# chaoting-sun/GCT-Plus

Hardware: AMD Instinct MI355X
Metric: SMILES/sec training step (vaetf, seq_len=80, d_model=512) (higher is better)
Workload: dtype f32

## Files before the change

gct_plus_amd/csrc/gemm.hip:

```cpp
#include <limits.h>
#include <stdlib.h>

#include <type_traits>

#include "common.h"

typedef float f32x16 __attribute__((ext_vector_type(16)));

namespace {

constexpr int BM = 128, BN = 128, BK = 32;
constexpr int TILE_FLOATS = BM * BK;

struct Seg3 {
  const float* p0;
  int64_t d1, d2;
};

struct GemmArgs {
  int64_t M, N, K;
  Seg3 a;
  int64_t lda;
  int64_t a_nper;
  Seg3 b;
// ... 930 lines not shown
#pragma unroll
    for (int rr = 0; rr < 4; ++rr) v[rr] = *reinterpret_cast<const float4*>(stg + (rg * 4 + rr) * 32 + c4 * 4);
    if (g.epi == EPI_SLAB) {
      float* sl = g.c0 + (int64_t)z * g.slab_stride;
#pragma unroll
      for (int rr = 0; rr < 4; ++rr)
        if (row0 + rr < g.M) *reinterpret_cast<float4*>(sl + (row0 + rr) * g.N + col0) = v[rr];
      return;
    }
    const bool q1 = col0 >= g.c_nper, q2 = col0 >= 2 * g.c_nper;
    const int64_t cloc = col0 - (q2 ? 2 * g.c_nper : (q1 ? g.c_nper : 0));
    float* cbase = g.c0 + (q2 ? g.c_d2 : (q1 ? g.c_d1 : 0));
    float4 bias = make_float4(0.f, 0.f, 0.f, 0.f);
    if (g.bias0) bias = *reinterpret_cast<const float4*>(g.bias0 + (q2 ? g.bias_d2 : (q1 ? g.bias_d1 : 0)) + cloc);
    ep.apply(v, row0, col0, cbase, cloc, bias);
  }
}


template <int TN, bool RAGGED = false>
__global__ __launch_bounds__(256) void gemm_f32_panel_kernel(const GemmArgs g) {
  constexpr int TM = 32, KC = 256, SD = KC + 4, NBL = TN / 4;
  extern __shared__ __attribute__((aligned(16))) float plds[];
  float* As = plds;
  float* Bs = plds + TM * SD;
  const int tid = threadIdx.x, lane = tid & 63, wave = tid >> 6, g4 = lane >> 4, c16 = lane & 15;
  const unsigned tiles_m = (unsigned)((g.M + TM - 1) / TM);
  const unsigned lid = gct_xcd_remap(blockIdx.x, gridDim.x);
  const int64_t m0 = (int64_t)(lid % tiles_m) * TM, n0 = (int64_t)(lid / tiles_m) * TN;
  const bool s1 = n0 >= g.b_nper, s2 = n0 >= 2 * g.b_nper;
  const float* bbase = g.b.p0 + (s2 ? g.b.d2 : (s1 ? g.b.d1 : 0)) + (n0 - (s2 ? 2 * g.b_nper : (s1 ? g.b_nper : 0))) * g.ldb;
  const float* abase = g.a.p0;
  uint32_t offa[8], offb[NBL];
#pragma unroll
  for (int i = 0; i < 8; ++i) {
    const int idx = tid + 256 * i, row = idx >> 6, c4 = idx & 63;
    int64_t r = m0 + row;
    if (r > g.M - 1) r = g.M - 1;
    offa[i] = (uint32_t)(r * g.lda + c4 * 4);
  }
#pragma unroll
  for (int i = 0; i < NBL; ++i) {
    const int idx = tid + 256 * i, c4 = idx & 63;
    int64_t row = idx >> 6;
    if (RAGGED && n0 + row > g.N - 1) row = g.N - 1 - n0;
    offb[i] = (uint32_t)(row * g.ldb + c4 * 4);
  }
  f32x4_t ra[8], rb[NBL];
  auto gload = [&](int64_t k0) {
#pragma unroll
    for (int i = 0; i < 8; ++i) ra[i] = *reinterpret_cast<const f32x4_t*>(abase + k0 + offa[i]);
#pragma unroll
    for (int i = 0; i < NBL; ++i) rb[i] = *reinterpret_cast<const f32x4_t*>(bbase + k0 + offb[i]);
  };
  auto lstore = [&]() {
#pragma unroll
    for (int i = 0; i < 8; ++i) {
      const int idx = tid + 256 * i;
      *reinterpret_cast<f32x4_t*>(As + (idx >> 6) * SD + (idx & 63) * 4) = ra[i];
    }
#pragma unroll
    for (int i = 0; i < NBL; ++i) {
      const int idx = tid + 256 * i;
      *reinterpret_cast<f32x4_t*>(Bs + (idx >> 6) * SD + (idx & 63) * 4) = rb[i];
    }
  };
  constexpr int NS = TN / 32;
  const int wm = (wave >> 1) * 16, wn = (wave & 1) * (TN / 2);
  f32x4_t acc[NS];
#pragma unroll
  for (int j = 0; j < NS; ++j) acc[j] = (f32x4_t){0.f, 0.f, 0.f, 0.f};
  const int64_t nch = g.K / KC;
  gload(0);
  lstore();
  __syncthreads();
  for (int64_t c = 0; c < nch; ++c) {
    if (c + 1 < nch) gload((c + 1) * KC);
    const float* ap = As + (wm + c16) * SD + g4 * 64;
#pragma unroll 4
    for (int j = 0; j < 16; ++j) {
      const float4 a4 = *reinterpret_cast<const float4*>(ap + 4 * j);
#pragma unroll
      for (int u = 0; u < NS; ++u) {
        const float4 b4 = *reinterpret_cast<const float4*>(Bs + (wn + 16 * u + c16) * SD + g4 * 64 + 4 * j);
        acc[u] = __builtin_amdgcn_mfma_f32_16x16x4f32(a4.x, b4.x, acc[u], 0, 0, 0);
        acc[u] = __builtin_amdgcn_mfma_f32_16x16x4f32(a4.y, b4.y, acc[u], 0, 0, 0);
        acc[u] = __builtin_amdgcn_mfma_f32_16x16x4f32(a4.z, b4.z, acc[u], 0, 0, 0);
        acc[u] = __builtin_amdgcn_mfma_f32_16x16x4f32(a4.w, b4.w, acc[u], 0, 0, 0);
      }
    }
    __syncthreads();
    if (c + 1 < nch) {
      lstore();
      __syncthreads();
    }
  }
  float* stg = plds + wave * (16 * 20);
  const FastEpi ep{g};
#pragma unroll
  for (int u = 0; u < NS; ++u) {
#pragma unroll
    for (int i = 0; i < 4; ++i) stg[(4 * g4 + i) * 20 + c16] = acc[u][i];
    __builtin_amdgcn_s_waitcnt(0xC07F);
    __builtin_amdgcn_wave_barrier();
    if (lane < 16) {
      const int pr = lane >> 2, pc = lane & 3;
      const int64_t row0 = m0 + wm + 4 * pr, col0 = n0 + wn + 16 * u + 4 * pc;
      if (RAGGED) {
        for (int rr = 0; rr < 4; ++rr)
          for (int cc = 0; cc < 4; ++cc)
            if (row0 + rr < g.M && col0 + cc < g.N)
              g.c0[(row0 + rr) * g.ldc + col0 + cc] = stg[(4 * pr + rr) * 20 + 4 * pc + cc] + (g.bias0 ? g.bias0[col0 + cc] : 0.f);
      } else if (row0 < g.M && col0 < g.N) {
        float4 v[4];
#pragma unroll
        for (int rr = 0; rr < 4; ++rr) v[rr] = *reinterpret_cast<const float4*>(stg + (4 * pr + rr) * 20 + 4 * pc);
        const bool q1 = col0 >= g.c_nper, q2 = col0 >= 2 * g.c_nper;
        const int64_t cloc = col0 - (q2 ? 2 * g.c_nper : (q1 ? g.c_nper : 0));
        float* cbase = g.c0 + (q2 ? g.c_d2 : (q1 ? g.c_d1 : 0));
        float4 bias = make_float4(0.f, 0.f, 0.f, 0.f);
        if (g.bias0) bias = *reinterpret_cast<const float4*>(g.bias0 + (q2 ? g.bias_d2 : (q1 ? g.bias_d1 : 0)) + cloc);
        ep.apply(v, row0, col0, cbase, cloc, bias);
      }
    }
    __builtin_amdgcn_s_waitcnt(0xC07F);
    __builtin_amdgcn_wave_barrier();
  }
}

template <int TN, bool RAGGED = false>
int launch_panel(const GemmArgs& g, hipStream_t st) {
  constexpr size_t LDS = (size_t)(32 + TN) * 260 * sizeof(float);
  static bool attr_set = false;
  if (!attr_set) {
    hipError_t e = hipFuncSetAttribute((const void*)gemm_f32_panel_kernel<TN, RAGGED>, hipFuncAttributeMaxDynamicSharedMemorySize, (int)LDS);
    if (e != hipSuccess) {
      gct_set_error("gemm_f32_panel: cannot reserve %zu bytes of LDS: %s", LDS, hipGetErrorString(e));
      return GCT_ERR_HIP;
    }
    attr_set = true;
  }
  const int64_t tiles = ((g.M + 31) / 32) * (RAGGED ? 1 : g.N / TN);
  hipLaunchKernelGGL((gemm_f32_panel_kernel<TN, RAGGED>), dim3((unsigned)tiles), dim3(256), LDS, st, g);
  GCT_LAUNCH_CHECK("gemm_f32_panel");
  return GCT_OK;
}

__global__ __launch_bounds__(256) void splitk_epilogue_kernel(const GemmArgs g, const float* slabs,
                                                              int nslab, int64_t slab_stride) {
  const int64_t pc = g.N / 4, pr = (g.M + 3) / 4;
  const int64_t idx = (int64_t)blockIdx.x * blockDim.x + threadIdx.x;
  if (idx >= pc * pr) return;
  const int64_t row0 = (idx / pc) * 4, col0 = (idx % pc) * 4;
  float4 v[4];
#pragma unroll
  for (int rr = 0; rr < 4; ++rr) {
    v[rr] = make_float4(0.f, 0.f, 0.f, 0.f);
    if (row0 + rr < g.M) {
      const float* p = slabs + (row0 + rr) * g.N + col0;
      for (int s = 0; s < nslab; ++s) {
        const float4 t = *reinterpret_cast<const float4*>(p + (int64_t)s * slab_stride);
        v[rr].x += t.x; v[rr].y += t.y; v[rr].z += t.z; v[rr].w += t.w;
      }
    }
  }
  const bool q1 = col0 >= g.c_nper, q2 = col0 >= 2 * g.c_nper;
  const int64_t cloc = col0 - (q2 ? 2 * g.c_nper : (q1 ? g.c_nper : 0));
  float* cbase = g.c0 + (q2 ? g.c_d2 : (q1 ? g.c_d1 : 0));
  float4 bias = make_float4(0.f, 0.f, 0.f, 0.f);
  if (g.bias0) bias = *reinterpret_cast<const float4*>(g.bias0 + (q2 ? g.bias_d2 : (q1 ? g.bias_d1 : 0)) + cloc);
  const FastEpi ep{g};
  ep.apply(v, row0, col0, cbase, cloc, bias);
}

int g_gemm_mode = -1;
int64_t g_gemm_launches[2] = {0, 0};
inline int gemm_mode() {
  if (g_gemm_mode < 0) {
    const char* e = getenv("GCT_GEMM_MODE");
    g_gemm_mode = (e && (e[0] == 'f' || e[0] == '0')) ? GCT_GEMM_F32 : GCT_GEMM_BF16X6;
  }
  return g_gemm_mode;
}

template <bool A_KC, bool B_KC>
bool fast_ok(const GemmArgs& g, bool vec) {
  auto seg_ok = [](int64_t nper, int64_t extent, int64_t gran) { return nper >= extent || nper % gran == 0; };
  return vec && g.K % BK == 0 && g.ksplit % BK == 0 && g.M >= 4 && g.N >= 4 &&
         (A_KC ? seg_ok(g.a_nper, g.K, BK) : (seg_ok(g.a_nper, g.M, BM) && g.M % 4 == 0)) &&
         (B_KC ? seg_ok(g.b_nper, g.N, BN) : (seg_ok(g.b_nper, g.K, BK) && g.N % 4 == 0)) &&
         g.N % 4 == 0 && g.ldc % 4 == 0 && gct_aligned16(g.c0) && g.c_d1 % 4 == 0 && g.c_d2 % 4 == 0 &&
         (g.c_nper >= g.N || g.c_nper % 4 == 0) && g.slab_stride % 4 == 0 &&
         (!g.bias0 || (gct_aligned16(g.bias0) && g.bias_d1 % 4 == 0 && g.bias_d2 % 4 == 0)) &&
         (!g.resid || gct_aligned16(g.resid)) && (!g.pre || gct_aligned16(g.pre)) &&
         (!g.pre_in || gct_aligned16(g.pre_in)) && 130 * g.lda < (1ll << 31) && 130 * g.ldb < (1ll << 31);
}


inline int64_t slab_bytes(int64_t s, int64_t rows, int64_t cols) {
  return s > 1 ? s * rows * cols * (int64_t)sizeof(float) : 0;
}

inline bool skinny_m(int64_t M, int64_t N) { return ((M + BM - 1) / BM) * ((N + BN - 1) / BN) < 192; }

int skinny_splits(int64_t M, int64_t N, int64_t K) {
  const int64_t tiles = ((M + 63) / 64) * ((N + 63) / 64);
  if (tiles <= 0) return 1;
  int64_t ns = 768 / tiles;
  if (ns > K / BK / 4) ns = K / BK / 4;
  return ns < 1 ? 1 : (int)ns;
}

int x6_tail_plan(int64_t M, int64_t N, int64_t K, int64_t* m1_out) {
  constexpr int64_t CUS = 256;
  const int64_t tm = (M + XBM - 1) / XBM, tn = (N + XBN - 1) / XBN, tiles = tm * tn;
  const int64_t rem = tiles % CUS;
  if (tiles <= CUS || rem == 0 || rem % tn != 0 || K % XBK != 0) return 1;
  const int64_t nkt = K / XBK;
  int best = 1;
  double cost = 1.0;
  const double o = 3.3;
  for (int s2 = 2; s2 <= 8 && nkt / s2 >= 2; ++s2) {
    const double c = (double)((rem * s2 + CUS - 1) / CUS) * (o + (double)nkt / s2) / (o + nkt) + 0.05;
    if (c < cost - 1e-9) { cost = c; best = s2; }
  }
  if (best == 1 || cost > 0.75) return 1;
  *m1_out = (tiles - rem) / tn * XBM;
  return best;
}

int x6_splitk_all_plan(int64_t M, int64_t N, int64_t K) {
  constexpr int64_t CUS = 256;
  const int64_t tiles = ((M + XBM - 1) / XBM) * ((N + XBN - 1) / XBN), nkt = K / XBK;
  if (tiles > CUS / 2 || K % XBK != 0 || nkt < 32 || M < 1024 || (nkt < 64 && M < 2048)) return 1;
  int64_t sp = CUS / tiles;
  if (sp > nkt / 8) sp = nkt / 8;
  if (sp > 8) sp = 8;
  return sp < 2 ? 1 : (int)sp;
}


inline int64_t x6s_tiles(int64_t M, int64_t N) { return ((M + SBM - 1) / SBM) * ((N + SBN - 1) / SBN); }

inline bool x6s_shape(const GemmArgs& g) {
  const int64_t big = ((g.M + XBM - 1) / XBM) * ((g.N + XBN - 1) / XBN), small = x6s_tiles(g.M, g.N), nkt = g.K / XBK;
  return big <= 160 && small >= 96 && small <= (nkt <= 16 ? 512 : 256) && nkt <= 32;
}

constexpr int64_t X6_TAIL_SMALL_MAX = 512;

constexpr int64_t PANEL32_MAX_TILES = 4096, PANEL64_MAX_TILES = 768;


static_assert(BK == XBK, "the fp32 and bf16x6 kernels split K at the same granularity");
GemmArgs slab_args(const GemmArgs& g, int splits, float* ws) {
  const int64_t nkt = g.K / BK;
  GemmArgs p = g;
  p.ksplit = ((nkt + splits - 1) / splits) * BK;
  p.nsplit = (int)((g.K + p.ksplit - 1) / p.ksplit);
  p.epi = EPI_SLAB; p.c0 = ws; p.ldc = g.N; p.slab_stride = g.M * g.N;
  p.c_d1 = p.c_d2 = 0; p.c_nper = INT64_MAX / 4; p.bias0 = nullptr; p.resid = nullptr; p.pre = nullptr; p.pre_in = nullptr;
  return p;
}

int launch_fixup(const GemmArgs& g, const GemmArgs& slabs, hipStream_t st, const char* name) {
  const int64_t patches = ((g.M + 3) / 4) * (g.N / 4);
  hipLaunchKernelGGL(splitk_epilogue_kernel, dim3((unsigned)((patches + 255) / 256)), dim3(256), 0, st, g,
                     (const float*)slabs.c0, slabs.nsplit, slabs.slab_stride);
  GCT_LAUNCH_CHECK(name);
  return GCT_OK;
}

template <int MODE, int NP>
int launch_x6_tail_split(const GemmArgs& g, hipStream_t st, float* ws, int64_t ws_bytes) {
  if (MODE == X6_WGRAD || g.nsplit != 1 || !ws || !gct_aligned16(ws)) return launch_x6<MODE, NP>(g, st);
  int64_t m1 = 0;
  const int best = x6_tail_plan(g.M, g.N, g.K, &m1);
  const int64_t m2 = g.M - m1, nkt = g.K / XBK;
  hipStreamCaptureStatus cap = hipStreamCaptureStatusNone;
  if (best == 1 || slab_bytes(best, m2, g.N) > ws_bytes ||
      hipStreamIsCapturing(st, &cap) != hipSuccess || cap != hipStreamCaptureStatusNone)
    return launch_x6<MODE, NP>(g, st);
  GemmArgs head = g;
  head.M = m1;
  int rc = launch_x6<MODE, NP>(head, st);
  if (rc) return rc;
  GemmArgs e = g;
  e.M = m2; e.row_base = g.row_base + m1;
  e.a.p0 += m1 * g.lda;
  e.c0 += m1 * g.ldc;
  if (e.resid) e.resid += m1 * g.ldc;
  if (e.pre) e.pre += m1 * g.ldc;
  if (e.pre_in && !(g.pre_rows > 0 && g.quad_map)) e.pre_in += m1 * g.ldc;
  if (nkt <= 32 && x6s_tiles(m2, g.N) <= X6_TAIL_SMALL_MAX) {
    if (MODE == X6_FWD && x6s_ok(e, true)) return launch_x6s<X6_FWD, NP>(e, st);
    if (MODE == X6_DGRAD && x6s_dgrad_ok(e, true)) return launch_x6s<X6_DGRAD, NP>(e, st);
  }
  const GemmArgs p = slab_args(e, best, ws);
  rc = launch_x6<MODE, NP>(p, st);
  if (rc) return rc;
  return launch_fixup(e, p, st, "x6 tail fix-up");
}

struct GemmRoute {
  enum Kind {
    X6S,
    X6_SPLITK_ALL,
    PANEL_THIN,
    PANEL32,
    PANEL64,
    F32_SMALL,
    X6,
    F32_FAST,
    F32_VEC,
    F32,
  } kind;
  int splits;
// ... 312 lines not shown
```

gct_plus_amd/csrc/norm.hip:

```cpp
#include "common.h"

namespace {

constexpr int MAXC = 8;

template <int NC>
__global__ __launch_bounds__(256) void norm_fwd_kernel(const float* __restrict__ x,
                                                       const float* __restrict__ alpha,
                                                       const float* __restrict__ bias, float* y,
                                                       float* mean_out, float* rstd_out,
                                                       int64_t rows, int d, float eps) {
  const int lane = threadIdx.x & 63, wave = threadIdx.x >> 6;
  const int64_t nwaves = (int64_t)gridDim.x * 4;
  float4 a[NC], b[NC];
#pragma unroll
  for (int c = 0; c < NC; ++c) {
    const int col = c * 256 + lane * 4;
    if (col < d) {
      a[c] = *reinterpret_cast<const float4*>(alpha + col);
      b[c] = *reinterpret_cast<const float4*>(bias + col);
    }
  }
  for (int64_t row = (int64_t)blockIdx.x * 4 + wave; row < rows; row += nwaves) {
    const float* xr = x + row * d;
    float4 v[NC];
    float s = 0.f;
#pragma unroll
    for (int c = 0; c < NC; ++c) {
      const int col = c * 256 + lane * 4;
      v[c] = make_float4(0.f, 0.f, 0.f, 0.f);
      if (col < d) {
        v[c] = *reinterpret_cast<const float4*>(xr + col);
        s += (v[c].x + v[c].y) + (v[c].z + v[c].w);
      }
    }
    const float mean = gct_wave_sum(s) / (float)d;
    float ss = 0.f;
#pragma unroll
    for (int c = 0; c < NC; ++c) {
      const int col = c * 256 + lane * 4;
      if (col < d) {
        v[c].x -= mean; v[c].y -= mean; v[c].z -= mean; v[c].w -= mean;
        ss += (v[c].x * v[c].x + v[c].y * v[c].y) + (v[c].z * v[c].z + v[c].w * v[c].w);
      }
    }
    const float var = gct_wave_sum(ss) / (float)(d - 1);
    const float rstd = 1.0f / (sqrtf(var) + eps);
    if (lane == 0) {
      mean_out[row] = mean;
      rstd_out[row] = rstd;
    }
    float* yr = y + row * d;
#pragma unroll
    for (int c = 0; c < NC; ++c) {
      const int col = c * 256 + lane * 4;
      if (col < d) {
        float4 o;
        o.x = a[c].x * (v[c].x * rstd) + b[c].x;
        o.y = a[c].y * (v[c].y * rstd) + b[c].y;
        o.z = a[c].z * (v[c].z * rstd) + b[c].z;
        o.w = a[c].w * (v[c].w * rstd) + b[c].w;
        *reinterpret_cast<float4*>(yr + col) = o;
      }
    }
  }
}

template <int NC>
__global__ __launch_bounds__(256) void norm_bwd_kernel(const float* __restrict__ dy,
                                                       const float* __restrict__ x,
                                                       const float* __restrict__ alpha,
                                                       const float* __restrict__ mean_in,
                                                       const float* __restrict__ rstd_in,
                                                       const float* __restrict__ dres, float* dx,
                                                       float* partial, int64_t rows, int d,
                                                       float eps, const int32_t* __restrict__ qmap,
                                                       int64_t src_rows, float* dropo, uint32_t thr, float dscale,
                                                       GctRng rng) {
  const int lane = threadIdx.x & 63, wave = threadIdx.x >> 6;
  const int64_t nwaves = (int64_t)gridDim.x * 4;
  float4 a[NC], pa[NC], pb[NC];
#pragma unroll
  for (int c = 0; c < NC; ++c) {
    const int col = c * 256 + lane * 4;
    a[c] = make_float4(0.f, 0.f, 0.f, 0.f);
    if (col < d) a[c] = *reinterpret_cast<const float4*>(alpha + col);
    pa[c] = make_float4(0.f, 0.f, 0.f, 0.f);
    pb[c] = make_float4(0.f, 0.f, 0.f, 0.f);
  }
  const int64_t nquads = (rows + 3) >> 2;
  for (int64_t quad = (int64_t)blockIdx.x * 4 + wave; quad < nquads; quad += nwaves) {
   uint4 db[NC][2];
   if (dropo) {
     const int64_t oq = qmap ? (int64_t)qmap[quad] : quad;
#pragma unroll
     for (int c = 0; c < NC; ++c) {
       const int col = c * 256 + lane * 4;
       db[c][0] = gct_drop_bits(rng, (uint32_t)(oq < 0 ? 0 : oq), (uint32_t)col);
       db[c][1] = gct_drop_bits(rng, (uint32_t)(oq < 0 ? 0 : oq), (uint32_t)col + 2);
     }
   }
   for (int e4 = 0; e4 < 4; ++e4) {
    const int64_t row = quad * 4 + e4;
    if (row >= rows) break;
    int64_t srow = row;
    if (qmap) {
      const int q = qmap[row >> 2];
      if (src_rows > 0) srow = (int64_t)q * 4 + (row & 3);
      if (q < 0 || (src_rows > 0 && srow >= src_rows)) {
        float* dr0 = dx + row * d;
#pragma unroll
        for (int c = 0; c < NC; ++c) {
          const int col = c * 256 + lane * 4;
          if (col < d) {
            *reinterpret_cast<float4*>(dr0 + col) = make_float4(0.f, 0.f, 0.f, 0.f);
            if (dropo) *reinterpret_cast<float4*>(dropo + row * d + col) = make_float4(0.f, 0.f, 0.f, 0.f);
          }
        }
        continue;
      }
    }
    const float mean = mean_in[srow], r = rstd_in[srow];
    const float* xr = x + srow * d;
    const float* gr = dy + row * d;
    float4 cx[NC], g[NC];
    float s1 = 0.f, s2 = 0.f;
#pragma unroll
    for (int c = 0; c < NC; ++c) {
      const int col = c * 256 + lane * 4;
      cx[c] = make_float4(0.f, 0.f, 0.f, 0.f);
      g[c] = cx[c];
      if (col < d) {
        float4 xv = *reinterpret_cast<const float4*>(xr + col);
        const float4 dv = *reinterpret_cast<const float4*>(gr + col);
        xv.x -= mean; xv.y -= mean; xv.z -= mean; xv.w -= mean;
        cx[c] = xv;
        pa[c].x += dv.x * xv.x * r; pa[c].y += dv.y * xv.y * r;
        pa[c].z += dv.z * xv.z * r; pa[c].w += dv.w * xv.w * r;
        pb[c].x += dv.x; pb[c].y += dv.y; pb[c].z += dv.z; pb[c].w += dv.w;
        g[c] = make_float4(dv.x * a[c].x, dv.y * a[c].y, dv.z * a[c].z, dv.w * a[c].w);
        s1 += (g[c].x + g[c].y) + (g[c].z + g[c].w);
        s2 += (g[c].x * xv.x + g[c].y * xv.y) + (g[c].z * xv.z + g[c].w * xv.w);
      }
    }
    s1 = gct_wave_sum(s1) / (float)d;
    s2 = gct_wave_sum(s2);
    const float sigma = 1.0f / r - eps;
    const float k2 = sigma > 0.f ? s2 * r * r / (sigma * (float)(d - 1)) : 0.f;
    float* dr = dx + row * d;
#pragma unroll
    for (int c = 0; c < NC; ++c) {
      const int col = c * 256 + lane * 4;
      if (col < d) {
        float4 o;
        o.x = r * (g[c].x - s1) - cx[c].x * k2;
        o.y = r * (g[c].y - s1) - cx[c].y * k2;
        o.z = r * (g[c].z - s1) - cx[c].z * k2;
        o.w = r * (g[c].w - s1) - cx[c].w * k2;
        if (dres) {
          const float4 e = *reinterpret_cast<const float4*>(dres + row * d + col);
          o.x += e.x; o.y += e.y; o.z += e.z; o.w += e.w;
        }
        *reinterpret_cast<float4*>(dr + col) = o;
        if (dropo) {
          const int e = e4;
          const uint4 b0 = db[c][0], b1 = db[c][1];
          float4 m;
          m.x = gct_drop_keep(b0, e, (uint32_t)col, thr) ? o.x * dscale : 0.f;
          m.y = gct_drop_keep(b0, e, (uint32_t)col + 1, thr) ? o.y * dscale : 0.f;
          m.z = gct_drop_keep(b1, e, (uint32_t)col + 2, thr) ? o.z * dscale : 0.f;
          m.w = gct_drop_keep(b1, e, (uint32_t)col + 3, thr) ? o.w * dscale : 0.f;
          *reinterpret_cast<float4*>(dropo + row * d + col) = m;
        }
      }
    }
   }
  }
  __shared__ float4 comb[4][64];
#pragma unroll
  for (int c = 0; c < NC; ++c) {
    const int col = c * 256 + lane * 4;
    for (int which = 0; which < 2; ++which) {
      __syncthreads();
      comb[wave][lane] = which == 0 ? pa[c] : pb[c];
      __syncthreads();
      if (wave == 0 && col < d) {
        float4 t = comb[0][lane];
        for (int w = 1; w < 4; ++w) {
          t.x += comb[w][lane].x; t.y += comb[w][lane].y;
          t.z += comb[w][lane].z; t.w += comb[w][lane].w;
        }
        *reinterpret_cast<float4*>(partial + ((int64_t)blockIdx.x * 2 + which) * d + col) = t;
      }
    }
  }
}

inline int norm_blocks(int64_t rows) {
  int64_t b = (rows + 3) / 4;
  if (b > 1024) b = 1024;
  if (b < 1) b = 1;
  return (int)b;
}

}

int gct_reduce_slabs_seg(const float* slabs, int nslab, int64_t stride, float* d0, float* d1,
                         float* d2, int64_t nper_elems, int64_t n, hipStream_t st);

#define NORM_DISPATCH(KERNEL, ...)                                                      \
  do {                                                                                  \
    const int nc = (d + 255) / 256;                                                     \
    if (nc <= 1) hipLaunchKernelGGL((KERNEL<1>), grid, dim3(256), 0, st, __VA_ARGS__);  \
    else if (nc <= 2) hipLaunchKernelGGL((KERNEL<2>), grid, dim3(256), 0, st, __VA_ARGS__); \
    else if (nc <= 4) hipLaunchKernelGGL((KERNEL<4>), grid, dim3(256), 0, st, __VA_ARGS__); \
    else hipLaunchKernelGGL((KERNEL<8>), grid, dim3(256), 0, st, __VA_ARGS__);          \
  } while (0)

extern "C" int gct_norm_fwd(const float* x, const float* alpha, const float* bias, float* y,
                            float* mean, float* rstd, int64_t rows, int d, float eps,
                            void* stream) {
  GCT_CHECK_ARG(x && alpha && bias && y && mean && rstd, "norm_fwd: null pointer");
  GCT_CHECK_ARG(rows >= 0 && d >= 4 && d % 4 == 0 && d <= 256 * MAXC, "norm_fwd: d=%d unsupported", d);
  GCT_CHECK_ARG(gct_aligned16(x) && gct_aligned16(y) && gct_aligned16(alpha) && gct_aligned16(bias),
                "norm_fwd: pointers must be 16-B aligned");
  if (rows == 0) return GCT_OK;
  hipStream_t st = (hipStream_t)stream;
  dim3 grid((unsigned)((rows + 3) / 4 > 8192 ? 8192 : (rows + 3) / 4));
  NORM_DISPATCH(norm_fwd_kernel, x, alpha, bias, y, mean, rstd, rows, d, eps);
  GCT_LAUNCH_CHECK("norm_fwd");
  return GCT_OK;
}

extern "C" int gct_norm_bwd(const float* dy, const float* x, const float* alpha, const float* mean,
                            const float* rstd, const float* dres, float* dx, float* dalpha,
                            float* dbias, float* ws, int64_t rows, int d, float eps,
                            const int32_t* quad_map, int64_t src_rows, float* drop_out, float p, uint64_t seed,
                            uint32_t site, void* stream) {
  GCT_CHECK_ARG(dy && x && alpha && mean && rstd && dx && dalpha && dbias && ws,
                "norm_bwd: null pointer");
  GCT_CHECK_ARG(!drop_out || (gct_aligned16(drop_out) && p >= 0.f && p < 1.f), "norm_bwd: bad dropout output");
  GCT_CHECK_ARG(!quad_map || (rows % 4 == 0 && src_rows >= 0), "norm_bwd: compacted rows come in quads");
  GCT_CHECK_ARG(rows >= 0 && d >= 4 && d % 4 == 0 && d <= 256 * MAXC, "norm_bwd: d=%d unsupported", d);
  GCT_CHECK_ARG(gct_aligned16(dy) && gct_aligned16(x) && gct_aligned16(dx) && gct_aligned16(alpha) &&
                    gct_aligned16(ws) && (!dres || gct_aligned16(dres)),
                "norm_bwd: pointers must be 16-B aligned");
  hipStream_t st = (hipStream_t)stream;
  const int nblk = norm_blocks(rows);
  dim3 grid((unsigned)nblk);
  NORM_DISPATCH(norm_bwd_kernel, dy, x, alpha, mean, rstd, dres, dx, ws, rows, d, eps, quad_map, src_rows, drop_out,
                gct_drop_threshold(p), 1.0f / (1.0f - p), gct_rng_make(seed, site));
  GCT_LAUNCH_CHECK("norm_bwd");
  return gct_reduce_slabs_seg(ws, nblk, (int64_t)2 * d, dalpha, dbias, nullptr, d, (int64_t)2 * d, st);
}
```

gct_plus_amd/csrc/reduce.hip:

```cpp
#include "common.h"

namespace {

template <int SL>
__device__ __forceinline__ void reduce_slabs_body(float4* red, const float* __restrict__ slabs, int nslab,
                                                  int64_t stride, float* d0, float* d1, float* d2, int64_t nper,
                                                  int64_t n4, int accumulate, unsigned bid, unsigned nblk) {
  constexpr int CW = 256 / SL;
  const int c = threadIdx.x % CW, sl = threadIdx.x / CW;
  for (int64_t base = (int64_t)bid * CW; base < n4; base += (int64_t)nblk * CW) {
    const int64_t i = base + c;
    float4 a = make_float4(0.f, 0.f, 0.f, 0.f);
    if (i < n4) {
      const float* src = slabs + i * 4;
      int s = sl;
      for (; s + 3 * SL < nslab; s += 4 * SL) {
        const float4 v0 = *reinterpret_cast<const float4*>(src + (int64_t)s * stride);
        const float4 v1 = *reinterpret_cast<const float4*>(src + (int64_t)(s + SL) * stride);
        const float4 v2 = *reinterpret_cast<const float4*>(src + (int64_t)(s + 2 * SL) * stride);
        const float4 v3 = *reinterpret_cast<const float4*>(src + (int64_t)(s + 3 * SL) * stride);
        a.x += (v0.x + v1.x) + (v2.x + v3.x);
        a.y += (v0.y + v1.y) + (v2.y + v3.y);
        a.z += (v0.z + v1.z) + (v2.z + v3.z);
        a.w += (v0.w + v1.w) + (v2.w + v3.w);
      }
      for (; s < nslab; s += SL) {
        const float4 v = *reinterpret_cast<const float4*>(src + (int64_t)s * stride);
        a.x += v.x; a.y += v.y; a.z += v.z; a.w += v.w;
      }
    }
    __syncthreads();
    red[threadIdx.x] = a;
    __syncthreads();
    if (sl == 0 && i < n4) {
      for (int k = 1; k < SL; ++k) {
        const float4 v = red[k * CW + c];
        a.x += v.x; a.y += v.y; a.z += v.z; a.w += v.w;
      }
      const int64_t e = i * 4;
      const bool g1 = e >= nper, g2 = e >= 2 * nper;
      float* d = (g2 ? d2 : (g1 ? d1 : d0)) + (e - (g2 ? 2 * nper : (g1 ? nper : 0)));
      if (accumulate) {
        const float4 o = *reinterpret_cast<const float4*>(d);
        a.x += o.x; a.y += o.y; a.z += o.z; a.w += o.w;
      }
      *reinterpret_cast<float4*>(d) = a;
    }
  }
}

template <int SL>
__global__ __launch_bounds__(256) void reduce_slabs_kernel(const float* __restrict__ slabs,
                                                           int nslab, int64_t stride, float* d0,
                                                           float* d1, float* d2, int64_t nper,
                                                           int64_t n4, int accumulate) {
  __shared__ float4 red[256];
  reduce_slabs_body<SL>(red, slabs, nslab, stride, d0, d1, d2, nper, n4, accumulate, blockIdx.x, gridDim.x);
}

struct ReduceRegion {
  const float* slabs;
  int64_t stride;
  float *d0, *d1, *d2;
  int64_t nper, n4;
};
__global__ __launch_bounds__(256) void reduce_slabs2_kernel(const ReduceRegion a, const ReduceRegion b, int nslab,
                                                            unsigned ga) {
  __shared__ float4 red[256];
  if (blockIdx.x < ga)
    reduce_slabs_body<4>(red, a.slabs, nslab, a.stride, a.d0, a.d1, a.d2, a.nper, a.n4, 0, blockIdx.x, ga);
  else
    reduce_slabs_body<64>(red, b.slabs, nslab, b.stride, b.d0, b.d1, b.d2, b.nper, b.n4, 0, blockIdx.x - ga,
                          gridDim.x - ga);
}

struct ReduceJob {
  const float* slabs;
  float *d0, *d1, *d2;
  int64_t stride, nper, n4;
  int32_t nslab, sl;
};
constexpr int RJ_MAX = 24;
struct ReduceJobs {
  ReduceJob j[RJ_MAX];
  uint32_t first[RJ_MAX + 1];
  int32_t n;
};
__global__ __launch_bounds__(256) void reduce_multi_kernel(const ReduceJobs a) {
  __shared__ float4 red[256];
  int k = 0;
#pragma unroll 1
  for (int i = 1; i < a.n; ++i)
    if (blockIdx.x >= a.first[i]) k = i;
  const ReduceJob& j = a.j[k];
  const unsigned bid = blockIdx.x - a.first[k], nblk = a.first[k + 1] - a.first[k];
  if (j.sl == 4) reduce_slabs_body<4>(red, j.slabs, j.nslab, j.stride, j.d0, j.d1, j.d2, j.nper, j.n4, 0, bid, nblk);
  else if (j.sl == 16) reduce_slabs_body<16>(red, j.slabs, j.nslab, j.stride, j.d0, j.d1, j.d2, j.nper, j.n4, 0, bid, nblk);
  else reduce_slabs_body<64>(red, j.slabs, j.nslab, j.stride, j.d0, j.d1, j.d2, j.nper, j.n4, 0, bid, nblk);
}

thread_local bool t_defer = false;
thread_local int t_njobs = 0;
thread_local ReduceJob t_jobs[4 * RJ_MAX];

inline unsigned rj_blocks(const ReduceJob& j) {
  const int cw = 256 / j.sl;
  int64_t g = (j.n4 + cw - 1) / cw;
  const int64_t cap = j.sl == 4 ? 8192 : 1024;
  return (unsigned)(g < 1 ? 1 : (g > cap ? cap : g));
}
int flush_jobs(hipStream_t st) {
  for (int base = 0; base < t_njobs; base += RJ_MAX) {
    ReduceJobs a;
    a.n = t_njobs - base < RJ_MAX ? t_njobs - base : RJ_MAX;
    unsigned nb = 0;
    for (int i = 0; i < a.n; ++i) {
      a.j[i] = t_jobs[base + i];
      a.first[i] = nb;
      nb += rj_blocks(a.j[i]);
    }
    for (int i = a.n; i <= RJ_MAX; ++i) a.first[i] = nb;
    hipLaunchKernelGGL(reduce_multi_kernel, dim3(nb), dim3(256), 0, st, a);
  }
  t_njobs = 0;
  GCT_LAUNCH_CHECK("reduce_multi");
  return GCT_OK;
}
inline bool defer_job(const float* slabs, int nslab, int64_t stride, float* d0, float* d1, float* d2, int64_t nper,
                      int64_t n4, int sl) {
  if (!t_defer || t_njobs >= 4 * RJ_MAX) return false;
  t_jobs[t_njobs++] = ReduceJob{slabs, d0, d1, d2, stride, nper, n4, nslab, sl};
  return true;
}

static int launch_reduce(const float* slabs, int nslab, int64_t stride, float* d0, float* d1,
                         float* d2, int64_t nper, int64_t n4, int accumulate, hipStream_t st) {
  auto grid = [&](int cw) {
    int64_t g = (n4 + cw - 1) / cw;
    return dim3((unsigned)(g < 1 ? 1 : (g > 8192 ? 8192 : g)));
  };
  const int sl = (n4 >= 16384 || nslab <= 4) ? 4 : ((n4 >= 1024 || nslab <= 16) ? 16 : 64);
  if (!accumulate && defer_job(slabs, nslab, stride, d0, d1, d2, nper, n4, sl)) return 0;
  if (accumulate && t_njobs > 0) flush_jobs(st);
  if (n4 >= 16384 || nslab <= 4)
    hipLaunchKernelGGL(reduce_slabs_kernel<4>, grid(64), dim3(256), 0, st, slabs, nslab, stride, d0,
                       d1, d2, nper, n4, accumulate);
  else if (n4 >= 1024 || nslab <= 16)
    hipLaunchKernelGGL(reduce_slabs_kernel<16>, grid(16), dim3(256), 0, st, slabs, nslab, stride,
                       d0, d1, d2, nper, n4, accumulate);
  else
    hipLaunchKernelGGL(reduce_slabs_kernel<64>, grid(4), dim3(256), 0, st, slabs, nslab, stride, d0,
                       d1, d2, nper, n4, accumulate);
  return 0;
}

__global__ __launch_bounds__(256) void reduce_slabs_scalar_kernel(const float* __restrict__ slabs,
                                                                  int nslab, int64_t stride,
                                                                  float* d0, float* d1, float* d2,
                                                                  int64_t nper, int64_t n,
                                                                  int accumulate) {
  for (int64_t e = (int64_t)blockIdx.x * blockDim.x + threadIdx.x; e < n;
       e += (int64_t)gridDim.x * blockDim.x) {
    float a = slabs[e];
    for (int s = 1; s < nslab; ++s) a += slabs[(int64_t)s * stride + e];
    const int q = (int)(e >= nper) + (int)(e >= 2 * nper);
    float* d = (q == 0 ? d0 : (q == 1 ? d1 : d2)) + (e - q * nper);
    *d = accumulate ? *d + a : a;
  }
}

__global__ __launch_bounds__(256) void colsum_partial_kernel(const float* y0, const float* y1,
                                                             const float* y2, int64_t ld,
                                                             int64_t M, int64_t nper, int64_t N,
                                                             int64_t rows_per_chunk,
                                                             float* partial) {
  const int64_t n = (int64_t)blockIdx.x * blockDim.x + threadIdx.x;
  if (n >= N) return;
  const int q = (int)(n >= nper) + (int)(n >= 2 * nper);
// ... 276 lines not shown
```

Before: 11000.

## Prefetch rows in norm kernels, batch slab loads in split-K and reductions

The layernorm forward kernel now handles two rows per wave, fuses their wave reductions and prefetches the next pair while the current one is reduced. The backward kernel software-pipelines its row loads, is specialized at compile time on whether dropout is present, and packs dropout keep bits ahead of use. The split-K epilogue and slab reduction issue more independent loads per iteration to raise memory-level parallelism. The extra registers from prefetching and wider unrolling may lower occupancy, and a waves-per-EU attribute is added to the backward kernel.

```diff
diff --git a/gct_plus_amd/csrc/gemm.hip b/gct_plus_amd/csrc/gemm.hip
--- a/gct_plus_amd/csrc/gemm.hip
+++ b/gct_plus_amd/csrc/gemm.hip
@@ -1106,17 +1106,38 @@
   const int64_t idx = (int64_t)blockIdx.x * blockDim.x + threadIdx.x;
   if (idx >= pc * pr) return;
   const int64_t row0 = (idx / pc) * 4, col0 = (idx % pc) * 4;
+  constexpr int FIX_S = 4;
   float4 v[4];
+  const float* p[4];
 #pragma unroll
   for (int rr = 0; rr < 4; ++rr) {
     v[rr] = make_float4(0.f, 0.f, 0.f, 0.f);
-    if (row0 + rr < g.M) {
-      const float* p = slabs + (row0 + rr) * g.N + col0;
-      for (int s = 0; s < nslab; ++s) {
-        const float4 t = *reinterpret_cast<const float4*>(p + (int64_t)s * slab_stride);
-        v[rr].x += t.x; v[rr].y += t.y; v[rr].z += t.z; v[rr].w += t.w;
+    p[rr] = slabs + (row0 + rr < g.M ? row0 + rr : row0) * g.N + col0;
+  }
+  int s = 0;
+  for (; s + FIX_S <= nslab; s += FIX_S) {
+    float4 t[FIX_S][4];
+#pragma unroll
+    for (int u = 0; u < FIX_S; ++u)
+#pragma unroll
+      for (int rr = 0; rr < 4; ++rr) t[u][rr] = *reinterpret_cast<const float4*>(p[rr] + (int64_t)(s + u) * slab_stride);
+#pragma unroll
+    for (int u = 0; u < FIX_S; ++u)
+#pragma unroll
+      for (int rr = 0; rr < 4; ++rr)
+        if (row0 + rr < g.M) {
+          v[rr].x += t[u][rr].x; v[rr].y += t[u][rr].y; v[rr].z += t[u][rr].z; v[rr].w += t[u][rr].w;
+        }
+  }
+  for (; s < nslab; ++s) {
+    float4 t[4];
+#pragma unroll
+    for (int rr = 0; rr < 4; ++rr) t[rr] = *reinterpret_cast<const float4*>(p[rr] + (int64_t)s * slab_stride);
+#pragma unroll
+    for (int rr = 0; rr < 4; ++rr)
+      if (row0 + rr < g.M) {
+        v[rr].x += t[rr].x; v[rr].y += t[rr].y; v[rr].z += t[rr].z; v[rr].w += t[rr].w;
       }
-    }
   }
   const bool q1 = col0 >= g.c_nper, q2 = col0 >= 2 * g.c_nper;
   const int64_t cloc = col0 - (q2 ? 2 * g.c_nper : (q1 ? g.c_nper : 0));
diff --git a/gct_plus_amd/csrc/norm.hip b/gct_plus_amd/csrc/norm.hip
--- a/gct_plus_amd/csrc/norm.hip
+++ b/gct_plus_amd/csrc/norm.hip
@@ -3,6 +3,15 @@
 namespace {
 
 constexpr int MAXC = 8;
+
+__device__ __forceinline__ void wave_sum2(float& u, float& v) {
+#pragma unroll
+  for (int o = 32; o > 0; o >>= 1) {
+    const float tu = __shfl_xor(u, o, 64), tv = __shfl_xor(v, o, 64);
+    u += tu;
+    v += tv;
+  }
+}
 
 template <int NC>
 __global__ __launch_bounds__(256) void norm_fwd_kernel(const float* __restrict__ x,
@@ -10,8 +19,26 @@
                                                        const float* __restrict__ bias, float* y,
                                                        float* mean_out, float* rstd_out,
                                                        int64_t rows, int d, float eps) {
-  const int lane = threadIdx.x & 63, wave = threadIdx.x >> 6;
+  const int lane = threadIdx.x & 63, wave = __builtin_amdgcn_readfirstlane(threadIdx.x >> 6);
   const int64_t nwaves = (int64_t)gridDim.x * 4;
+  const int64_t npairs = (rows + 1) >> 1;
+  int64_t pair = (int64_t)blockIdx.x * 4 + wave;
+  float4 n0[NC], n1[NC];
+  auto fetch = [&](int64_t p) {
+    const int64_t r0 = 2 * p, r1 = r0 + 1 < rows ? r0 + 1 : rows - 1;
+    const float *x0 = x + r0 * d, *x1 = x + r1 * d;
+#pragma unroll
+    for (int c = 0; c < NC; ++c) {
+      const int col = c * 256 + lane * 4;
+      n0[c] = make_float4(0.f, 0.f, 0.f, 0.f);
+      n1[c] = n0[c];
+      if (col < d) {
+        n0[c] = *reinterpret_cast<const float4*>(x0 + col);
+        n1[c] = *reinterpret_cast<const float4*>(x1 + col);
+      }
+    }
+  };
+  if (pair < npairs) fetch(pair);
   float4 a[NC], b[NC];
 #pragma unroll
   for (int c = 0; c < NC; ++c) {
@@ -21,63 +48,76 @@
       b[c] = *reinterpret_cast<const float4*>(bias + col);
     }
   }
-  for (int64_t row = (int64_t)blockIdx.x * 4 + wave; row < rows; row += nwaves) {
-    const float* xr = x + row * d;
-    float4 v[NC];
-    float s = 0.f;
-#pragma unroll
-    for (int c = 0; c < NC; ++c) {
-      const int col = c * 256 + lane * 4;
-      v[c] = make_float4(0.f, 0.f, 0.f, 0.f);
+  for (; pair < npairs; pair += nwaves) {
+    const int64_t row0 = 2 * pair, row1 = row0 + 1;
+    float4 v0[NC], v1[NC];
+    float s0 = 0.f, s1 = 0.f;
+#pragma unroll
+    for (int c = 0; c < NC; ++c) {
+      const int col = c * 256 + lane * 4;
+      v0[c] = n0[c];
+      v1[c] = n1[c];
       if (col < d) {
-        v[c] = *reinterpret_cast<const float4*>(xr + col);
-        s += (v[c].x + v[c].y) + (v[c].z + v[c].w);
-      }
-    }
-    const float mean = gct_wave_sum(s) / (float)d;
-    float ss = 0.f;
+        s0 += (v0[c].x + v0[c].y) + (v0[c].z + v0[c].w);
+        s1 += (v1[c].x + v1[c].y) + (v1[c].z + v1[c].w);
+      }
+    }
+    if (pair + nwaves < npairs) fetch(pair + nwaves);
+    wave_sum2(s0, s1);
+    const float mean0 = s0 / (float)d, mean1 = s1 / (float)d;
+    float ss0 = 0.f, ss1 = 0.f;
 #pragma unroll
     for (int c = 0; c < NC; ++c) {
       const int col = c * 256 + lane * 4;
       if (col < d) {
-        v[c].x -= mean; v[c].y -= mean; v[c].z -= mean; v[c].w -= mean;
-        ss += (v[c].x * v[c].x + v[c].y * v[c].y) + (v[c].z * v[c].z + v[c].w * v[c].w);
-      }
-    }
-    const float var = gct_wave_sum(ss) / (float)(d - 1);
-    const float rstd = 1.0f / (sqrtf(var) + eps);
+        v0[c].x -= mean0; v0[c].y -= mean0; v0[c].z -= mean0; v0[c].w -= mean0;
+        ss0 += (v0[c].x * v0[c].x + v0[c].y * v0[c].y) + (v0[c].z * v0[c].z + v0[c].w * v0[c].w);
+        v1[c].x -= mean1; v1[c].y -= mean1; v1[c].z -= mean1; v1[c].w -= mean1;
+        ss1 += (v1[c].x * v1[c].x + v1[c].y * v1[c].y) + (v1[c].z * v1[c].z + v1[c].w * v1[c].w);
+      }
+    }
+    wave_sum2(ss0, ss1);
+    const float var0 = ss0 / (float)(d - 1), var1 = ss1 / (float)(d - 1);
+    const float rstd0 = 1.0f / (sqrtf(var0) + eps), rstd1 = 1.0f / (sqrtf(var1) + eps);
+    const bool two = row1 < rows;
     if (lane == 0) {
-      mean_out[row] = mean;
-      rstd_out[row] = rstd;
-    }
-    float* yr = y + row * d;
+      mean_out[row0] = mean0;
+      rstd_out[row0] = rstd0;
+      if (two) {
+        mean_out[row1] = mean1;
+        rstd_out[row1] = rstd1;
+      }
+    }
+    float *y0 = y + row0 * d, *y1 = y + row1 * d;
 #pragma unroll
     for (int c = 0; c < NC; ++c) {
       const int col = c * 256 + lane * 4;
       if (col < d) {
         float4 o;
-        o.x = a[c].x * (v[c].x * rstd) + b[c].x;
-        o.y = a[c].y * (v[c].y * rstd) + b[c].y;
-        o.z = a[c].z * (v[c].z * rstd) + b[c].z;
-        o.w = a[c].w * (v[c].w * rstd) + b[c].w;
-        *reinterpret_cast<float4*>(yr + col) = o;
-      }
-    }
-  }
-}
-
-template <int NC>
-__global__ __launch_bounds__(256) void norm_bwd_kernel(const float* __restrict__ dy,
-                                                       const float* __restrict__ x,
-                                                       const float* __restrict__ alpha,
-                                                       const float* __restrict__ mean_in,
-                                                       const float* __restrict__ rstd_in,
-                                                       const float* __restrict__ dres, float* dx,
-                                                       float* partial, int64_t rows, int d,
-                                                       float eps, const int32_t* __restrict__ qmap,
-                                                       int64_t src_rows, float* dropo, uint32_t thr, float dscale,
-                                                       GctRng rng) {
-  const int lane = threadIdx.x & 63, wave = threadIdx.x >> 6;
+        o.x = a[c].x * (v0[c].x * rstd0) + b[c].x;
+        o.y = a[c].y * (v0[c].y * rstd0) + b[c].y;
+        o.z = a[c].z * (v0[c].z * rstd0) + b[c].z;
+        o.w = a[c].w * (v0[c].w * rstd0) + b[c].w;
+        *reinterpret_cast<float4*>(y0 + col) = o;
+        if (two) {
+          o.x = a[c].x * (v1[c].x * rstd1) + b[c].x;
+          o.y = a[c].y * (v1[c].y * rstd1) + b[c].y;
+          o.z = a[c].z * (v1[c].z * rstd1) + b[c].z;
+          o.w = a[c].w * (v1[c].w * rstd1) + b[c].w;
+          *reinterpret_cast<float4*>(y1 + col) = o;
+        }
+      }
+    }
+  }
+}
+
+template <int NC, bool DROP>
+__global__ __launch_bounds__(256) __attribute__((amdgpu_waves_per_eu(NC <= 2 ? 4 : 1)))
+void norm_bwd_kernel(const float* dy, const float* __restrict__ x, const float* __restrict__ alpha,
+                     const float* __restrict__ mean_in, const float* __restrict__ rstd_in, const float* dres,
+                     float* dx, float* partial, int64_t rows, int d, float eps, const int32_t* __restrict__ qmap,
+                     int64_t src_rows, float* dropo, uint32_t thr, float dscale, GctRng rng) {
+  const int lane = threadIdx.x & 63, wave = __builtin_amdgcn_readfirstlane(threadIdx.x >> 6);
   const int64_t nwaves = (int64_t)gridDim.x * 4;
   float4 a[NC], pa[NC], pb[NC];
 #pragma unroll
@@ -89,92 +129,138 @@
     pb[c] = make_float4(0.f, 0.f, 0.f, 0.f);
   }
   const int64_t nquads = (rows + 3) >> 2;
-  for (int64_t quad = (int64_t)blockIdx.x * 4 + wave; quad < nquads; quad += nwaves) {
-   uint4 db[NC][2];
-   if (dropo) {
-     const int64_t oq = qmap ? (int64_t)qmap[quad] : quad;
-#pragma unroll
-     for (int c = 0; c < NC; ++c) {
-       const int col = c * 256 + lane * 4;
-       db[c][0] = gct_drop_bits(rng, (uint32_t)(oq < 0 ? 0 : oq), (uint32_t)col);
-       db[c][1] = gct_drop_bits(rng, (uint32_t)(oq < 0 ? 0 : oq), (uint32_t)col + 2);
-     }
-   }
+  float4 xn[NC], dn[NC], en[NC];
+  float mean_n = 0.f, r_n = 0.f;
+  int kind_n = 0;
+  auto fetch = [&](int64_t quad, int e4) {
+    kind_n = 0;
+    if (quad >= nquads) return;
+    const int64_t row = quad * 4 + e4;
+    int64_t srow = row;
+    kind_n = 2;
+    if (qmap) {
+      const int q = qmap[quad];
+      if (src_rows > 0) srow = (int64_t)q * 4 + e4;
+      if (q < 0 || (src_rows > 0 && srow >= src_rows)) kind_n = 1;
+    }
+    if (kind_n == 2) {
+      mean_n = mean_in[srow];
+      r_n = rstd_in[srow];
+      const float* xr = x + srow * d;
+      const float* gr = dy + row * d;
+      const float* er = dres + row * d;
+#pragma unroll
+      for (int c = 0; c < NC; ++c) {
+        const int col = c * 256 + lane * 4;
+        if (col < d) {
+          xn[c] = *reinterpret_cast<const float4*>(xr + col);
+          dn[c] = *reinterpret_cast<const float4*>(gr + col);
+          if (dres) en[c] = *reinterpret_cast<const float4*>(er + col);
+        }
+      }
+    }
+  };
+  uint32_t keep[4] = {0u, 0u, 0u, 0u};
+  auto draw = [&](int64_t quad) {
+    const int64_t oq = qmap ? (int64_t)qmap[quad] : quad;
+#pragma unroll
+    for (int e = 0; e < 4; ++e) keep[e] = 0u;
+#pragma unroll
+    for (int c = 0; c < NC; ++c) {
+      const int col = c * 256 + lane * 4;
+      const uint4 b0 = gct_drop_bits(rng, (uint32_t)(oq < 0 ? 0 : oq), (uint32_t)col);
+      const uint4 b1 = gct_drop_bits(rng, (uint32_t)(oq < 0 ? 0 : oq), (uint32_t)col + 2);
+#pragma unroll
+      for (int e = 0; e < 4; ++e)
+        keep[e] |= ((uint32_t)gct_drop_keep(b0, e, (uint32_t)col, thr) << (4 * c)) |
+                   ((uint32_t)gct_drop_keep(b0, e, (uint32_t)col + 1, thr) << (4 * c + 1)) |
+                   ((uint32_t)gct_drop_keep(b1, e, (uint32_t)col + 2, thr) << (4 * c + 2)) |
+                   ((uint32_t)gct_drop_keep(b1, e, (uint32_t)col + 3, thr) << (4 * c + 3));
+    }
+  };
+  int64_t quad = (int64_t)blockIdx.x * 4 + wave;
+  fetch(quad, 0);
+  if (DROP && quad < nquads) draw(quad);
+  for (; quad < nquads; quad += nwaves) {
+#pragma unroll
    for (int e4 = 0; e4 < 4; ++e4) {
     const int64_t row = quad * 4 + e4;
     if (row >= rows) break;
-    int64_t srow = row;
-    if (qmap) {
-      const int q = qmap[row >> 2];
-      if (src_rows > 0) srow = (int64_t)q * 4 + (row & 3);
-      if (q < 0 || (src_rows > 0 && srow >= src_rows)) {
-        float* dr0 = dx + row * d;
-#pragma unroll
-        for (int c = 0; c < NC; ++c) {
-          const int col = c * 256 + lane * 4;
-          if (col < d) {
-            *reinterpret_cast<float4*>(dr0 + col) = make_float4(0.f, 0.f, 0.f, 0.f);
-            if (dropo) *reinterpret_cast<float4*>(dropo + row * d + col) = make_float4(0.f, 0.f, 0.f, 0.f);
+    const int kind = kind_n;
+    const float mean = mean_n, r = r_n;
+    float4 xc[NC], dc[NC], ec[NC];
+#pragma unroll
+    for (int c = 0; c < NC; ++c) {
+      xc[c] = xn[c];
+      dc[c] = dn[c];
+      ec[c] = en[c];
+    }
+    if (e4 < 3 && row + 1 < rows) fetch(quad, e4 + 1);
+    else fetch(quad + nwaves, 0);
+    if (kind == 1) {
+      float* dr0 = dx + row * d;
+#pragma unroll
+      for (int c = 0; c < NC; ++c) {
+        const int col = c * 256 + lane * 4;
+        if (col < d) {
+          *reinterpret_cast<float4*>(dr0 + col) = make_float4(0.f, 0.f, 0.f, 0.f);
+          if (DROP) *reinterpret_cast<float4*>(dropo + row * d + col) = make_float4(0.f, 0.f, 0.f, 0.f);
+        }
+      }
+    } else {
+      float4 cx[NC], g[NC];
+      float s1 = 0.f, s2 = 0.f;
+#pragma unroll
+      for (int c = 0; c < NC; ++c) {
+        const int col = c * 256 + lane * 4;
+        cx[c] = make_float4(0.f, 0.f, 0.f, 0.f);
+        g[c] = cx[c];
+        if (col < d) {
+          float4 xv = xc[c];
+          const float4 dv = dc[c];
+          xv.x -= mean; xv.y -= mean; xv.z -= mean; xv.w -= mean;
+          cx[c] = xv;
+          pa[c].x += dv.x * xv.x * r; pa[c].y += dv.y * xv.y * r;
+          pa[c].z += dv.z * xv.z * r; pa[c].w += dv.w * xv.w * r;
+          pb[c].x += dv.x; pb[c].y += dv.y; pb[c].z += dv.z; pb[c].w += dv.w;
+          g[c] = make_float4(dv.x * a[c].x, dv.y * a[c].y, dv.z * a[c].z, dv.w * a[c].w);
+          s1 += (g[c].x + g[c].y) + (g[c].z + g[c].w);
+          s2 += (g[c].x * xv.x + g[c].y * xv.y) + (g[c].z * xv.z + g[c].w * xv.w);
+        }
+      }
+      wave_sum2(s1, s2);
+      s1 = s1 / (float)d;
+      const float sigma = 1.0f / r - eps;
+      const float k2 = sigma > 0.f ? s2 * r * r / (sigma * (float)(d - 1)) : 0.f;
+      float* dr = dx + row * d;
+#pragma unroll
+      for (int c = 0; c < NC; ++c) {
+        const int col = c * 256 + lane * 4;
+        if (col < d) {
+          float4 o;
+          o.x = r * (g[c].x - s1) - cx[c].x * k2;
+          o.y = r * (g[c].y - s1) - cx[c].y * k2;
+          o.z = r * (g[c].z - s1) - cx[c].z * k2;
+          o.w = r * (g[c].w - s1) - cx[c].w * k2;
+          if (dres) {
+            const float4 e = ec[c];
+            o.x += e.x; o.y += e.y; o.z += e.z; o.w += e.w;
           }
-        }
-        continue;
-      }
-    }
-    const float mean = mean_in[srow], r = rstd_in[srow];
-    const float* xr = x + srow * d;
-    const float* gr = dy + row * d;
-    float4 cx[NC], g[NC];
-    float s1 = 0.f, s2 = 0.f;
-#pragma unroll
-    for (int c = 0; c < NC; ++c) {
-      const int col = c * 256 + lane * 4;
-      cx[c] = make_float4(0.f, 0.f, 0.f, 0.f);
-      g[c] = cx[c];
-      if (col < d) {
-        float4 xv = *reinterpret_cast<const float4*>(xr + col);
-        const float4 dv = *reinterpret_cast<const float4*>(gr + col);
-        xv.x -= mean; xv.y -= mean; xv.z -= mean; xv.w -= mean;
-        cx[c] = xv;
-        pa[c].x += dv.x * xv.x * r; pa[c].y += dv.y * xv.y * r;
-        pa[c].z += dv.z * xv.z * r; pa[c].w += dv.w * xv.w * r;
-        pb[c].x += dv.x; pb[c].y += dv.y; pb[c].z += dv.z; pb[c].w += dv.w;
-        g[c] = make_float4(dv.x * a[c].x, dv.y * a[c].y, dv.z * a[c].z, dv.w * a[c].w);
-        s1 += (g[c].x + g[c].y) + (g[c].z + g[c].w);
-        s2 += (g[c].x * xv.x + g[c].y * xv.y) + (g[c].z * xv.z + g[c].w * xv.w);
-      }
-    }
-    s1 = gct_wave_sum(s1) / (float)d;
-    s2 = gct_wave_sum(s2);
-    const float sigma = 1.0f / r - eps;
-    const float k2 = sigma > 0.f ? s2 * r * r / (sigma * (float)(d - 1)) : 0.f;
-    float* dr = dx + row * d;
-#pragma unroll
-    for (int c = 0; c < NC; ++c) {
-      const int col = c * 256 + lane * 4;
-      if (col < d) {
-        float4 o;
-        o.x = r * (g[c].x - s1) - cx[c].x * k2;
-        o.y = r * (g[c].y - s1) - cx[c].y * k2;
-        o.z = r * (g[c].z - s1) - cx[c].z * k2;
-        o.w = r * (g[c].w - s1) - cx[c].w * k2;
-        if (dres) {
-          const float4 e = *reinterpret_cast<const float4*>(dres + row * d + col);
-          o.x += e.x; o.y += e.y; o.z += e.z; o.w += e.w;
-        }
-        *reinterpret_cast<float4*>(dr + col) = o;
-        if (dropo) {
-          const int e = e4;
-          const uint4 b0 = db[c][0], b1 = db[c][1];
-          float4 m;
-          m.x = gct_drop_keep(b0, e, (uint32_t)col, thr) ? o.x * dscale : 0.f;
-          m.y = gct_drop_keep(b0, e, (uint32_t)col + 1, thr) ? o.y * dscale : 0.f;
-          m.z = gct_drop_keep(b1, e, (uint32_t)col + 2, thr) ? o.z * dscale : 0.f;
-          m.w = gct_drop_keep(b1, e, (uint32_t)col + 3, thr) ? o.w * dscale : 0.f;
-          *reinterpret_cast<float4*>(dropo + row * d + col) = m;
+          *reinterpret_cast<float4*>(dr + col) = o;
+          if (DROP) {
+            const uint32_t k = keep[e4] >> (4 * c);
+            float4 m;
+            m.x = (k & 1u) ? o.x * dscale : 0.f;
+            m.y = (k & 2u) ? o.y * dscale : 0.f;
+            m.z = (k & 4u) ? o.z * dscale : 0.f;
+            m.w = (k & 8u) ? o.w * dscale : 0.f;
+            *reinterpret_cast<float4*>(dropo + row * d + col) = m;
+          }
         }
       }
     }
    }
+   if (DROP && quad + nwaves < nquads) draw(quad + nwaves);
   }
   __shared__ float4 comb[4][64];
 #pragma unroll
@@ -203,18 +289,26 @@
   return (int)b;
 }
 
+inline int norm_fwd_blocks(int64_t rows) {
+  const int64_t units = (((rows + 1) >> 1) + 3) / 4, cap = 2048;
+  const int64_t iters = (units + cap - 1) / cap;
+  const int64_t b = iters > 0 ? (units + iters - 1) / iters : 1;
+  return (int)(b < 1 ? 1 : b);
+}
+
 }
 
 int gct_reduce_slabs_seg(const float* slabs, int nslab, int64_t stride, float* d0, float* d1,
                          float* d2, int64_t nper_elems, int64_t n, hipStream_t st);
 
-#define NORM_DISPATCH(KERNEL, ...)                                                      \
-  do {                                                                                  \
-    const int nc = (d + 255) / 256;                                                     \
-    if (nc <= 1) hipLaunchKernelGGL((KERNEL<1>), grid, dim3(256), 0, st, __VA_ARGS__);  \
-    else if (nc <= 2) hipLaunchKernelGGL((KERNEL<2>), grid, dim3(256), 0, st, __VA_ARGS__); \
-    else if (nc <= 4) hipLaunchKernelGGL((KERNEL<4>), grid, dim3(256), 0, st, __VA_ARGS__); \
-    else hipLaunchKernelGGL((KERNEL<8>), grid, dim3(256), 0, st, __VA_ARGS__);          \
+#define NORM_TAIL(...) __VA_ARGS__
+#define NORM_DISPATCH(KERNEL, TAIL, ...)                                                               \
+  do {                                                                                                 \
+    const int nc = (d + 255) / 256;                                                                    \
+    if (nc <= 1) hipLaunchKernelGGL((KERNEL<1 NORM_TAIL TAIL>), grid, dim3(256), 0, st, __VA_ARGS__);  \
+    else if (nc <= 2) hipLaunchKernelGGL((KERNEL<2 NORM_TAIL TAIL>), grid, dim3(256), 0, st, __VA_ARGS__); \
+    else if (nc <= 4) hipLaunchKernelGGL((KERNEL<4 NORM_TAIL TAIL>), grid, dim3(256), 0, st, __VA_ARGS__); \
+    else hipLaunchKernelGGL((KERNEL<8 NORM_TAIL TAIL>), grid, dim3(256), 0, st, __VA_ARGS__);          \
   } while (0)
 
 extern "C" int gct_norm_fwd(const float* x, const float* alpha, const float* bias, float* y,
@@ -226,8 +320,8 @@
                 "norm_fwd: pointers must be 16-B aligned");
   if (rows == 0) return GCT_OK;
   hipStream_t st = (hipStream_t)stream;
-  dim3 grid((unsigned)((rows + 3) / 4 > 8192 ? 8192 : (rows + 3) / 4));
-  NORM_DISPATCH(norm_fwd_kernel, x, alpha, bias, y, mean, rstd, rows, d, eps);
+  dim3 grid((unsigned)norm_fwd_blocks(rows));
+  NORM_DISPATCH(norm_fwd_kernel, (), x, alpha, bias, y, mean, rstd, rows, d, eps);
   GCT_LAUNCH_CHECK("norm_fwd");
   return GCT_OK;
 }
@@ -248,8 +342,12 @@
   hipStream_t st = (hipStream_t)stream;
   const int nblk = norm_blocks(rows);
   dim3 grid((unsigned)nblk);
-  NORM_DISPATCH(norm_bwd_kernel, dy, x, alpha, mean, rstd, dres, dx, ws, rows, d, eps, quad_map, src_rows, drop_out,
-                gct_drop_threshold(p), 1.0f / (1.0f - p), gct_rng_make(seed, site));
+  if (drop_out)
+    NORM_DISPATCH(norm_bwd_kernel, (, true), dy, x, alpha, mean, rstd, dres, dx, ws, rows, d, eps, quad_map, src_rows,
+                  drop_out, gct_drop_threshold(p), 1.0f / (1.0f - p), gct_rng_make(seed, site));
+  else
+    NORM_DISPATCH(norm_bwd_kernel, (, false), dy, x, alpha, mean, rstd, dres, dx, ws, rows, d, eps, quad_map, src_rows,
+                  drop_out, gct_drop_threshold(p), 1.0f / (1.0f - p), gct_rng_make(seed, site));
   GCT_LAUNCH_CHECK("norm_bwd");
   return gct_reduce_slabs_seg(ws, nblk, (int64_t)2 * d, dalpha, dbias, nullptr, d, (int64_t)2 * d, st);
 }
diff --git a/gct_plus_amd/csrc/reduce.hip b/gct_plus_amd/csrc/reduce.hip
--- a/gct_plus_amd/csrc/reduce.hip
+++ b/gct_plus_amd/csrc/reduce.hip
@@ -1,6 +1,22 @@
 #include "common.h"
 
 namespace {
+
+template <int G, int SL>
+__device__ __forceinline__ void slab_groups(float4& a, const float* __restrict__ src, int64_t stride, int& s, int nslab) {
+  for (; s + (4 * G - 1) * SL < nslab; s += 4 * G * SL) {
+    float4 v[4 * G];
+#pragma unroll
+    for (int u = 0; u < 4 * G; ++u) v[u] = *reinterpret_cast<const float4*>(src + (int64_t)(s + u * SL) * stride);
+#pragma unroll
+    for (int g = 0; g < G; ++g) {
+      a.x += (v[4 * g].x + v[4 * g + 1].x) + (v[4 * g + 2].x + v[4 * g + 3].x);
+      a.y += (v[4 * g].y + v[4 * g + 1].y) + (v[4 * g + 2].y + v[4 * g + 3].y);
+      a.z += (v[4 * g].z + v[4 * g + 1].z) + (v[4 * g + 2].z + v[4 * g + 3].z);
+      a.w += (v[4 * g].w + v[4 * g + 1].w) + (v[4 * g + 2].w + v[4 * g + 3].w);
+    }
+  }
+}
 
 template <int SL>
 __device__ __forceinline__ void reduce_slabs_body(float4* red, const float* __restrict__ slabs, int nslab,
@@ -14,16 +30,8 @@
     if (i < n4) {
       const float* src = slabs + i * 4;
       int s = sl;
-      for (; s + 3 * SL < nslab; s += 4 * SL) {
-        const float4 v0 = *reinterpret_cast<const float4*>(src + (int64_t)s * stride);
-        const float4 v1 = *reinterpret_cast<const float4*>(src + (int64_t)(s + SL) * stride);
-        const float4 v2 = *reinterpret_cast<const float4*>(src + (int64_t)(s + 2 * SL) * stride);
-        const float4 v3 = *reinterpret_cast<const float4*>(src + (int64_t)(s + 3 * SL) * stride);
-        a.x += (v0.x + v1.x) + (v2.x + v3.x);
-        a.y += (v0.y + v1.y) + (v2.y + v3.y);
-        a.z += (v0.z + v1.z) + (v2.z + v3.z);
-        a.w += (v0.w + v1.w) + (v2.w + v3.w);
-      }
+      slab_groups<2, SL>(a, src, stride, s, nslab);
+      slab_groups<1, SL>(a, src, stride, s, nslab);
       for (; s < nslab; s += SL) {
         const float4 v = *reinterpret_cast<const float4*>(src + (int64_t)s * stride);
         a.x += v.x; a.y += v.y; a.z += v.z; a.w += v.w;
```

After: 11000 (median of 6 runs). No clear change (+0.0%).
